# codeonwort/Software-Raytracing

Hardware: AMD Instinct MI355X
Metric: Mrays/sec (primary+secondary) + frame time, Cornell Box 1080p 64spp (higher is better)
Workload: dtype f32

## Files before the change

### include/raylib_amd.h

```cpp
#ifndef RAYLIB_AMD_H
#define RAYLIB_AMD_H

#include "raylib_types.h"

#ifdef __cplusplus
extern "C" {
#endif

typedef struct RaylibAMDStats {
	uint64_t rays;
	uint64_t nodesVisited;
	uint64_t trisTested;
	uint64_t shadedHits;
	uint64_t texFetches;
	uint64_t cameraSamples;
	uint64_t pixels;
	double   kernelMs;
	double   traceKernelMs;
	double   wallMs;
	uint32_t traceLaunches;
	uint32_t numNodes;
	uint32_t numTriangles;
	uint32_t bvhDepth;
	uint64_t waveTrips;
// ... 156 lines not shown

RAYLIB_API int32_t RaylibAMD_VerifyExactMath(int32_t which, uint64_t* outMismatches, uint64_t* outFirstBits);
RAYLIB_API int32_t RaylibAMD_VerifyLazyRefl(uint32_t n, uint64_t seed, uint64_t* outEvents, uint64_t* outUnsafe, uint64_t* outGuardFailed);
RAYLIB_API int32_t RaylibAMD_VerifyLazyPdf(uint32_t n, uint64_t seed, uint64_t* outEvents, uint64_t* outWrong, uint64_t* outRefused);

RAYLIB_API int32_t RaylibAMD_SceneNumTriangles(SceneHandle scene);
RAYLIB_API int32_t RaylibAMD_SceneNumMaterials(SceneHandle scene);
RAYLIB_API int32_t RaylibAMD_SceneNumTextures(SceneHandle scene);
RAYLIB_API void    RaylibAMD_SceneExportTriangles(SceneHandle scene, void* outTriangles);
RAYLIB_API void    RaylibAMD_SceneExportMaterials(SceneHandle scene, void* outMaterials);
RAYLIB_API void    RaylibAMD_SceneTextureSize(SceneHandle scene, int32_t index, int32_t* outW, int32_t* outH);
RAYLIB_API void    RaylibAMD_SceneExportTexture(SceneHandle scene, int32_t index, float* outRGBA);
RAYLIB_API void    RaylibAMD_SceneGetSun(SceneHandle scene, float outIlluminance[3], float outDirection[3]);
RAYLIB_API int32_t RaylibAMD_SceneBVHInfo(SceneHandle scene, uint32_t* outNodes, uint32_t* outDepth, float* outSahCost);
RAYLIB_API int32_t RaylibAMD_SceneBVH4Info(SceneHandle scene, uint32_t* outNodes4, uint32_t* outWorstCaseStack);
RAYLIB_API int32_t RaylibAMD_SceneBVH8Info(SceneHandle scene, uint32_t* outNodes8, uint32_t* outLevels, float* outSteps4, float* outSteps8);
RAYLIB_API int32_t RaylibAMD_SceneWalk8Host(SceneHandle scene, const float* rays, int32_t count, float tMin, const float* tMax, float* outT, uint32_t* outSteps);
RAYLIB_API int32_t RaylibAMD_SceneWalkStackHost(SceneHandle scene, int32_t tree, const float* rays, int32_t count, float tMin, int32_t capacity, float* outT, uint32_t* outHighWater);
RAYLIB_API int32_t RaylibAMD_SceneLeafListInfo(SceneHandle scene, uint32_t* outMaxTrianglesPerLeaf);
RAYLIB_API int32_t RaylibAMD_ScenePlain(SceneHandle scene);
RAYLIB_API int32_t RaylibAMD_LastTracePlain(void);
RAYLIB_API int32_t RaylibAMD_SceneLazyRefl(SceneHandle scene);
RAYLIB_API int32_t RaylibAMD_LastTraceLazy(void);
typedef struct RaylibAMDRenderPlan {
	int32_t pathTrace;
	int32_t stack, prims;
	int32_t poolK;
	int32_t tree;
	int32_t lstack;
	int32_t lds;
	int32_t plain;
	uint32_t pathsPerWave, treeWidth, nodeBytes;
	int32_t keepNodes4, keepNodes4f;
	int32_t eagerTree;
	uint32_t batch, sampleCount, blocks, stackStride, jobChunk, heads, jobsPerHead, guideShift;
	uint64_t jobs;
	int32_t lazy;
	int32_t reserved;
} RaylibAMDRenderPlan;
RAYLIB_API int32_t RaylibAMD_PlanRender(SceneHandle scene, const RendererSettings* settings, int32_t hasSky, int32_t numCUs, int32_t workgroupsPerCU, RaylibAMDRenderPlan* out);
#define RAYLIB_AMD_MAX_VIEWS 64
RAYLIB_API int32_t RaylibAMD_RenderViews(const RendererSettings* settings, SceneHandle scene,
        const CameraHandle* cameras, int32_t count, const ImageHandle* outImages);
RAYLIB_API int32_t RaylibAMD_RenderViewsDevice(const RendererSettings* settings, SceneHandle scene,
        const CameraHandle* cameras, int32_t count, void* outDevice);
RAYLIB_API int32_t RaylibAMD_PlanViews(SceneHandle scene, const RendererSettings* settings, const CameraHandle* cameras, int32_t count, int32_t hasSky,
// ... 43 lines not shown
```

### software-raytracing_amd/csrc/rl_abi.cc

```cpp
#include "raylib.h"
#include "raylib_amd.h"
#include "rl_host.h"
#include "rl_plan.h"
#include "rl_progressive.h"
#include "rl_lightmap.h"
#include "raylib_amd_rng.h"

#include <math.h>
#include <stddef.h>
#include <stdio.h>
#include <stdlib.h>
#include <string.h>
#include <algorithm>

using namespace rl;

namespace {

template <typename T>
struct Registry {
	std::mutex mu;
	std::vector<T*> items;
	void add(T* p) { std::lock_guard<std::mutex> lk(mu); items.push_back(p); }
	bool eraseFirst(T* p) {
// ... 1040 lines not shown
	return WalkStackHost(s->bvh, s->triangles, s->spheres, s->cubes, tree, rays, count, tMin, capacity, outT, outHighWater) ? 1 : -1;
}
int32_t RaylibAMD_SceneLeafListInfo(SceneHandle sh, uint32_t* maxPerLeaf)
{
	Scene* s = (Scene*)sh;
	if (!s || !s->finalized) return 0;
	int32_t leaves = 0; uint32_t most = 0;
	for (const DNode4& n : s->bvh.leafList) for (int k = 0; k < 4; ++k) if (n.child[k] != DNODE_EMPTY) { ++leaves; most = std::max(most, (((uint32_t)~n.child[k]) & LEAF_COUNT_MASK) + 1u); }
	if (maxPerLeaf) *maxPerLeaf = most;
	return leaves;
}
int32_t RaylibAMD_ScenePlain(SceneHandle sh)
{
	Scene* s = (Scene*)sh;
	return (s && s->finalized && ScenePlain(*s)) ? 1 : 0;
}
int32_t RaylibAMD_LastTracePlain(void) { return DeviceLastTracePlain(); }
int32_t RaylibAMD_SceneLazyRefl(SceneHandle sh)
{
	Scene* s = (Scene*)sh;
	return (s && s->finalized && SceneLazyRefl(*s)) ? 1 : 0;
}
int32_t RaylibAMD_LastTraceLazy(void) { return DeviceLastTraceLazy(); }
int32_t RaylibAMD_PlanRender(SceneHandle sh, const RendererSettings* settings, int32_t hasSky, int32_t numCUs, int32_t workgroupsPerCU, RaylibAMDRenderPlan* out)
{
	Scene* s = (Scene*)sh;
	if (!s || !s->finalized || !settings || !out || numCUs < 1) return 0;
	memset(out, 0, sizeof(*out));
	const RenderKnobs knobs = ReadRenderKnobs();
	const TracePlan t = PlanTrace(*s, *settings, hasSky != 0, knobs);
	if (!t.ok) return -1;
	out->pathTrace = t.pathTrace; out->stack = t.stack; out->prims = t.prims; out->poolK = t.poolK; out->tree = t.tree; out->lstack = t.lstack; out->lds = t.lds; out->plain = t.plain; out->lazy = t.lazy ? 1 : 0;
	out->pathsPerWave = t.pathsPerWave; out->treeWidth = t.treeWidth; out->nodeBytes = t.nodeBytes;
	out->keepNodes4 = t.keepNodes4; out->keepNodes4f = t.keepNodes4f; out->eagerTree = t.eagerTree;
	const uint32_t cells = ((settings->viewportWidth + 7) / 8) * ((settings->viewportHeight + 7) / 8);
	const uint32_t spp = (uint32_t)(settings->samplesPerPixel > 1 ? settings->samplesPerPixel : 1);
	const LaunchPlan L = PlanLaunch(cells, cells, spp, 0, numCUs, workgroupsPerCU, t, knobs);
	out->batch = L.batch; out->sampleCount = L.sampleCount; out->blocks = L.blocks; out->stackStride = L.stackStride; out->jobChunk = L.jobChunk;
	out->heads = L.heads; out->jobsPerHead = L.jobsPerHead; out->guideShift = L.guideShift; out->jobs = L.jobs;
	return 1;
}
int32_t RaylibAMD_PlanViews(SceneHandle sh, const RendererSettings* settings, const CameraHandle* cameras, int32_t count, int32_t hasSky,
                           int32_t numCUs, int32_t workgroupsPerCU, RaylibAMDRenderPlan* out, uint8_t* outCellEmpty)
{
	Scene* s = (Scene*)sh;
	if (!out || numCUs < 1 || !ViewsArgsValid("RaylibAMD_PlanViews", settings, s, cameras, count, nullptr)) return 0;
// ... 81 lines not shown
```

### software-raytracing_amd/csrc/rl_device.h

```cpp
#pragma once

#include <stdint.h>

namespace rl {

#define DNODE_EMPTY ((int32_t)0x80000000)
enum : uint32_t { LEAF_FIRST_SHIFT = 6, LEAF_KIND_SHIFT = 4, LEAF_KIND_MASK = 3u, LEAF_ALPHA_BIT = 8u, LEAF_COUNT_MASK = 7u };
struct alignas(64) DNode {
	float lmin[3], lmax[3];
	float rmin[3], rmax[3];
	int32_t left, right;
	int32_t pad0, pad1;
};
static_assert(sizeof(DNode) == 64, "DNode");

struct alignas(128) DNode4 {
	float lo[3][4];
	float hi[3][4];
	int32_t child[4];
	uint32_t pad[4];
};
static_assert(sizeof(DNode4) == 128, "DNode4");

struct alignas(64) DNode4Q {
// ... 156 lines not shown
	float    emptyL[3];
	uint32_t emptySky;
	uint32_t magicSamples;
	uint32_t magicCellsX;
	uint64_t seedMixed;
	DCamera camera;
};

#define RL_MAX_VIEWS 64
struct DViews {
	const DCamera* cameras;
	uint32_t cellsPerView;
	uint32_t magicCellsPerView;
};

#define RL_LIT_CHUNK 64u
#define RL_LIT_CTL 16u
#define RL_LAZY_ROUGHNESS_MIN 0x1p-10f
#define RL_LAZY_ROUGHNESS_MAX 1.0f
#define RL_LAZY_COLOR_MAX 16.0f
#define RL_LAZY_MAX_PATH 4096
#define RL_LAZY_REC_EXACT_SP 0x40000000
#define RL_LAZY_REC_MAT(w) (__float_as_int(w) & ~RL_LAZY_REC_EXACT_SP)
struct DLitList {
	float* entries;
	uint32_t* ctl;
	uint32_t numChunks;
	uint32_t pad;
};

}
```

### software-raytracing_amd/csrc/rl_host.h

```cpp
#pragma once

#include "raylib_types.h"
#include "raylib_amd.h"
#include "rl_device.h"

#include <math.h>
#include <stdint.h>
#include <memory>
#include <mutex>
#include <string>
#include <vector>

namespace rl {

struct f3 { float x, y, z; };
inline f3 F3(float x, float y, float z) { f3 r; r.x = x; r.y = y; r.z = z; return r; }
inline f3 operator+(f3 a, f3 b) { return F3(a.x + b.x, a.y + b.y, a.z + b.z); }
inline f3 operator-(f3 a, f3 b) { return F3(a.x - b.x, a.y - b.y, a.z - b.z); }
inline f3 operator*(f3 a, f3 b) { return F3(a.x * b.x, a.y * b.y, a.z * b.z); }
inline f3 operator*(f3 a, float t) { return F3(a.x * t, a.y * t, a.z * t); }
inline f3 operator*(float t, f3 a) { return F3(a.x * t, a.y * t, a.z * t); }
inline f3 operator-(f3 a) { return F3(-a.x, -a.y, -a.z); }
inline float dot(f3 a, f3 b) { return a.x * b.x + a.y * b.y + a.z * b.z; }
inline f3 cross(f3 a, f3 b) { return F3(a.y * b.z - a.z * b.y, -(a.x * b.z - a.z * b.x), a.x * b.y - a.y * b.x); }
// ... 153 lines not shown
	DCamera camera;
	uint64_t seed;
	uint32_t cellFirst, cellStride;
	bool cellMajor = false;
	int slot = 0;
	void* outDevice;
	bool callerOwnsOut = false;
	float* outHostRGBA;
};
bool DeviceAvailable();
int DeviceNumRanks();
float ParseDecimalFloat(const char* token);
constexpr uint64_t kMaxImagePixels = 1ull << 28;
inline bool PlausibleImageSize(uint64_t w, uint64_t h, uint64_t fileBytes, uint64_t maxPixelsPerByte)
{
	return w > 0 && h > 0 && w <= 65535 && h <= 65535 && w * h <= kMaxImagePixels && w * h <= (fileBytes + 64) * maxPixelsPerByte;
}
bool DecodeJPEG(const std::vector<uint8_t>& data, uint32_t& w, uint32_t& h, std::vector<uint8_t>& rgba);
bool DecodeTGA(const std::vector<uint8_t>& data, uint32_t& w, uint32_t& h, std::vector<uint8_t>& rgba);
bool EncodeJPEG(uint32_t w, uint32_t h, const uint8_t* rgbTopDown, std::vector<uint8_t>& out);
bool DeviceRender(Scene& scene, const RenderRequest& req, RaylibAMDStats& stats);
bool DeviceRenderViews(Scene& scene, const RenderRequest& req, const DCamera* cameras, uint32_t count, void* outDevice, void* const* imagePixels, RaylibAMDStats& stats);
int32_t DeviceLastTraceLazy();
int32_t DeviceLastTracePlain();
bool DeviceDrain(RaylibAMDStats* outLastStats);
void DeviceOwnStats();
bool DeviceClosestHit(Scene& scene, const float* rays, int32_t n, float tMin, void* outHits);
bool DeviceTraceRays(Scene& scene, int32_t kind, const void* rays, int32_t n, float rayTime, void* out, int32_t* outPrim, bool hostMem, void* stream,
                     RaylibAMDStats& stats);
constexpr uint64_t RL_RADIANCE_STACK_BUDGET = 256ull << 20;
constexpr int32_t RL_RADIANCE_MAX_PATH = 32768;
bool DeviceTraceRadiance(Scene& scene, const RaylibAMDRadianceParams& prm, uint64_t seed, const void* rays, int32_t n, float* out, bool hostMem, void* stream,
                         RaylibAMDStats& stats);
constexpr uint64_t RL_GATHER_SAMPLE_BUDGET = 256ull << 20;
constexpr uint64_t RL_GATHER_MAX_SLOTS = 1ull << 28;
constexpr uint64_t RL_GATHER_TIMED = 4096;
bool DeviceGather(Scene& scene, int32_t kind, const RaylibAMDRadianceParams& prm, uint64_t seed, const void* points, int32_t n, float* out, bool hostMem, void* stream,
                  RaylibAMDStats& stats);
int64_t LightmapPointsHost(const Scene& scene, const RaylibAMDLightmapParams& P, int32_t triFirst, int32_t triCount, const float* uv,
                           RaylibAMDGatherPoint* outPoints, uint32_t* outTexel, int64_t capacity);
int64_t DeviceLightmapPoints(Scene& scene, const RaylibAMDLightmapParams& P, int32_t triFirst, int32_t triCount, const float* uv,
                             RaylibAMDGatherPoint* outPoints, uint32_t* outTexel, int64_t capacity);
bool DeviceBakeLightmap(Scene& scene, const RaylibAMDLightmapParams& P, int32_t triFirst, int32_t triCount, const RaylibAMDRadianceParams& prm, uint64_t seed,
                        const float* uv, float* out, uint8_t* outCoverage, bool hostMem, void* stream, RaylibAMDStats& stats,
                        const RaylibAMDLightmapFilterParams* filter = nullptr, const float* in = nullptr);
struct LmFilterInv { float invC[8], invN, invP[8]; };
// ... 33 lines not shown
```

### software-raytracing_amd/csrc/rl_kernels.h

```cpp
#pragma once

#include "rl_dev_jobs.h"
#include "rl_dev_pool.h"

namespace rl {

#ifndef RL_QUEUE_SPIN_LIMIT
#define RL_QUEUE_SPIN_LIMIT 0
#endif
#ifndef RL_TRACE_MIN_WAVES
#define RL_TRACE_MIN_WAVES 4
#endif
#define RL_TRACE_ARGS const DRenderParams, const DSceneView, const SkyRot, SampleRGB* __restrict__, float* __restrict__, unsigned long long* __restrict__, unsigned int* __restrict__
template <int STACK, bool PRIMS, bool FULL, int LDS = 0, bool PLAIN = false>
__global__ void __launch_bounds__(RL_BLOCK, (STACK <= 32 ? RL_TRACE_MIN_WAVES : 2)) k_trace(RL_TRACE_ARGS);
template <int STACK, bool PRIMS, bool FULL, int LDS = 0, bool PLAIN = false>
__global__ void __launch_bounds__(RL_BLOCK, (STACK <= 32 ? RL_TRACE_MIN_WAVES : 2)) k_trace_views(RL_TRACE_ARGS, const DViews);
#define RL_TRACE_INSTANCES(X) \
	X(16, false, false, 0, false) X(16, false, true, 0, false) X(16, false, true, 1, false) X(16, false, true, 2, false) X(16, false, true, 2, true) \
	X(32, false, false, 0, false) X(32, false, true, 0, false) X(32, true, false, 0, false) X(32, true, true, 0, false) \
	X(64, false, false, 0, false) X(64, false, true, 0, false) X(64, true, false, 0, false) X(64, true, true, 0, false)
#define RL_K_TRACE(a, b, c, d, e) template __global__ void k_trace<a, b, c, d, e>(RL_TRACE_ARGS);
#define RL_K_TRACE_VIEWS(a, b, c, d, e) template __global__ void k_trace_views<a, b, c, d, e>(RL_TRACE_ARGS, const DViews);
RL_TRACE_INSTANCES(extern RL_K_TRACE)
RL_TRACE_INSTANCES(extern RL_K_TRACE_VIEWS)
template <int STACK, bool PRIMS, bool FULL, int LDS, bool PLAIN>
__global__ void __launch_bounds__(RL_BLOCK, (STACK <= 32 ? RL_TRACE_MIN_WAVES : 2)) k_trace_lazy(RL_TRACE_ARGS, const DLitList);
#define RL_TRACE_LAZY_INSTANCES(X) X(16, false, true, 2, true)
#define RL_K_TRACE_LAZY(a, b, c, d, e) template __global__ void k_trace_lazy<a, b, c, d, e>(RL_TRACE_ARGS, const DLitList);
RL_TRACE_LAZY_INSTANCES(extern RL_K_TRACE_LAZY)
__global__ void __launch_bounds__(RL_BLOCK) k_fold_lit(const DSceneView S, const DLitList LL, SampleRGB* __restrict__ samples);

template <int STACK, bool PRIMS, int K, int LSTACK = STACK, int WIDE = 0>
__global__ void __launch_bounds__(RL_BLOCK, (PoolOcc<LSTACK, PRIMS, K>::kBlocks)) k_trace_pool(RL_TRACE_ARGS);
template <int STACK, bool PRIMS, int K, int LSTACK = STACK, int WIDE = 0>
__global__ void __launch_bounds__(RL_BLOCK, (PoolOcc<LSTACK, PRIMS, K>::kBlocks)) k_trace_pool_views(RL_TRACE_ARGS, const DViews);
#define RL_POOL_INSTANCES(X) \
	X(16, false, 2, 16, 0) X(16, false, 3, 16, 0) X(16, false, 4, 16, 0) X(32, false, 2, 32, 0) X(32, false, 3, 32, 0) X(32, false, 4, 32, 0) \
	X(32, false, 2, 4, 0) X(32, false, 2, RL_POOL_SHORT_LSTACK, 0) \
	X(32, false, 2, 32, 1) X(64, false, 2, 32, 1) X(32, false, 2, RL_POOL_SHORT_LSTACK, 1) X(64, false, 2, RL_POOL_SHORT_LSTACK, 1) \
	X(2 * RL_POOL8_MAXLEVELS, false, 2, RL_POOL8_LSTACK, 3)
#define RL_K_TRACE_POOL(a, b, c, d, e) template __global__ void k_trace_pool<a, b, c, d, e>(RL_TRACE_ARGS);
#define RL_K_TRACE_POOL_VIEWS(a, b, c, d, e) template __global__ void k_trace_pool_views<a, b, c, d, e>(RL_TRACE_ARGS, const DViews);
RL_POOL_INSTANCES(extern RL_K_TRACE_POOL_VIEWS)
RL_POOL_INSTANCES(extern RL_K_TRACE_POOL)

__global__ void __launch_bounds__(RL_BLOCK)
k_resolve(const DRenderParams P, const DSceneView S, const SkyRot R, const SampleRGB* __restrict__ samples, float4* __restrict__ accum, float4* __restrict__ out, int firstBatch, int lastBatch);
__global__ void __launch_bounds__(RL_BLOCK)
k_resolve_views(const DRenderParams Pb, const DSceneView S, const SkyRot R, const SampleRGB* __restrict__ samples, float4* __restrict__ accum, float4* __restrict__ out,
                int firstBatch, int lastBatch, const DViews V);
#define RL_AOV_ARGS const DRenderParams, const DSceneView, float4* __restrict__, unsigned long long* __restrict__
template <int STACK, bool PRIMS> __global__ void __launch_bounds__(RL_BLOCK) k_aov(RL_AOV_ARGS);
template <int STACK, bool PRIMS> __global__ void __launch_bounds__(RL_BLOCK) k_aov_views(RL_AOV_ARGS, const DViews);
// ... 125 lines not shown
```

### software-raytracing_amd/csrc/rl_plan.cc

```cpp
#include "rl_plan.h"

#include <algorithm>
#include <atomic>
#include <cmath>
#include <cstring>
#include <stdlib.h>

namespace rl {

RenderKnobs ReadRenderKnobs()
{
	RenderKnobs k;
	auto flag = [](const char* name) { const char* e = getenv(name); return e ? (atoi(e) != 0 ? 1 : 0) : -1; };
	if (const char* e = getenv("RAYLIB_POOL")) { const int v = atoi(e); k.pool = (v == 2 || v == 3 || v == 4) ? v : 0; }
	if (const char* e = getenv("RAYLIB_POOL_MIN_TRIS")) k.poolMinTris = (uint32_t)atoi(e);
	if (const char* e = getenv("RAYLIB_POOL_SHORT_STACK")) { const int v = atoi(e); k.poolShortStack = (v == 0 || v == 4) ? v : 1; }
	k.bvh4 = flag("RAYLIB_BVH4"); k.bvh8 = flag("RAYLIB_BVH8");
	k.ldsScene = flag("RAYLIB_LDS_SCENE"); k.leafList = flag("RAYLIB_LEAF_LIST"); k.plainKernel = flag("RAYLIB_PLAIN_KERNEL");
	if (const char* e = getenv("RAYLIB_SAMPLE_BATCH")) k.sampleBatch = std::max(0, atoi(e));
	if (const char* e = getenv("RAYLIB_SAMPLE_BUFFER_GIB")) k.sampleBufferGiB = std::max(0, atoi(e));
	if (const char* e = getenv("RAYLIB_JOB_CHUNK")) k.jobChunk = std::max(0, atoi(e));
	if (const char* e = getenv("RAYLIB_JOB_HEADS")) k.jobHeads = std::max(1, atoi(e));
	if (const char* e = getenv("RAYLIB_GUIDED")) k.guided = atoi(e);
	if (const char* e = getenv("RAYLIB_BLOCKS_PER_CU")) k.blocksPerCU = std::max(0, atoi(e));
	if (const char* e = getenv("RAYLIB_CULL_CELLS")) k.cullCells = atoi(e);
	k.lazyRefl = flag("RAYLIB_LAZY_REFL");
	if (const char* e = getenv("RAYLIB_LIT_LIST")) k.litList = std::max(0ll, atoll(e));
	if (const char* e = getenv("RAYLIB_QUERY_TREE")) { const int v = atoi(e); k.queryTree = (v == 2 || v == 4 || v == 8) ? v : 0; }
	if (const char* e = getenv("RAYLIB_GATHER_BATCH")) k.gatherBatch = std::max(0, atoi(e));
	return k;
}

namespace {

TracePlan Pick(const Scene& sc, const RendererSettings& st, bool hasSky, const RenderKnobs& k, bool say)
{
	TracePlan p;
	const BVH& b = sc.bvh;
	const size_t ntri = sc.triangles.size();
	p.prims = !sc.spheres.empty() || !sc.cubes.empty();
	if (b.depth > 64) {
		if (say) Log("Raylib_Render: BVH depth %u exceeds the traversal stack (64)", b.depth);
		p.ok = false;
		return p;
	}
	p.stack = (b.depth <= 16 && !p.prims) ? 16 : b.depth <= 32 ? 32 : 64;
	p.pathTrace = st.renderMode == RAYLIB_RENDERMODE_Default;
	if (!p.pathTrace) return p;
	const bool hasNodes4 = !b.nodes4.empty(), hasNodes8 = !b.nodes8.empty();

// ... 224 lines not shown
```

### software-raytracing_amd/csrc/rl_plan.h

```cpp
#pragma once

#include "rl_host.h"

namespace rl {

#define RL_POOL_DEFAULT_MIN_TRIS 256u
#define RL_FLOAT_BOX_MAX_TRIS 4096u

struct RenderKnobs {
	int pool = -1;
	uint32_t poolMinTris = RL_POOL_DEFAULT_MIN_TRIS;
	int poolShortStack = -1;
	int bvh4 = -1, bvh8 = -1;
	int ldsScene = -1, leafList = -1, plainKernel = -1;
	int sampleBatch = 0, sampleBufferGiB = 0;
	int jobChunk = -1;
	int jobHeads = 0;
	int guided = 0;
	int blocksPerCU = 0;
	int cullCells = 1;
	int queryTree = 0;
	int gatherBatch = 0;
	int lazyRefl = -1;
	long long litList = -1;
};
RenderKnobs ReadRenderKnobs();

enum PlanTree : int32_t { TREE_NONE = 0, TREE_BVH2 = 1, TREE_BOX4 = 2, TREE_GRID4 = 3, TREE_WIDE8 = 4 };

struct TracePlan {
	bool ok = true;
	bool pathTrace = true;
	int stack = 16;
	bool prims = false;
	int poolK = 0;
	int32_t tree = TREE_BVH2;
	int lstack = 0;
	int lds = 0;
	bool plain = false;
	bool lazy = false;
	uint32_t pathsPerWave = 64, treeWidth = 2, nodeBytes = 64;
	bool keepNodes4 = true, keepNodes4f = true;
	int32_t eagerTree = TREE_NONE;
};
TracePlan PlanTrace(const Scene& sc, const RendererSettings& st, bool hasSky, const RenderKnobs& knobs);
int32_t EagerTree(const Scene& sc);

// ... 43 lines not shown
```

### software-raytracing_amd/csrc/rl_render_lazy.hip

```cpp


#include "rl_kernels.h"

namespace rl {

#define RL_VIEWS_TWIN 0
#define RL_LAZY_REFL 1
#include "rl_k_trace.inl"
#undef RL_LAZY_REFL
#undef RL_VIEWS_TWIN

__global__ void __launch_bounds__(RL_BLOCK)
k_fold_lit(const DSceneView S, const DLitList LL, SampleRGB* __restrict__ samples)
{
	RL_MATH_PROLOGUE();
	const uint32_t lane = threadIdx.x & 63u;
	const uint32_t waves = gridDim.x * (RL_BLOCK / 64u);
	const uint32_t used = min(LL.ctl[0], LL.numChunks);
	for (uint32_t chunk = (blockIdx.x * RL_BLOCK + threadIdx.x) >> 6; chunk < used; chunk += waves) {
		if (lane >= min(LL.ctl[RL_LIT_CTL + chunk], RL_LIT_CHUNK)) continue;
		const float4* e = (const float4*)LL.entries + ((size_t)chunk * RL_LIT_CHUNK + lane) * RL_LIT_STRIDE;
		const float4 h0 = e[0];
		const int nrec = __float_as_int(e[1].x);
		V3 L = v3(h0.x, h0.y, h0.z);
		#pragma nounroll
		for (int k = nrec - 1; k >= 0; --k) {
			const float4 r0 = e[2 + 2 * k], r1 = e[3 + 2 * k];
			L = FoldLazyVertex(LoadMat(S, RL_LAZY_REC_MAT(r1.w)), r0, r1, L);
		}
		samples[__float_as_uint(h0.w)] = make_sample(L.x, L.y, L.z);
	}
}

__device__ __forceinline__ uint32_t LazySweepEvent(unsigned long long seed, uint32_t i, Rng& g, V3& Wo, float& u0, float& u1, float& rough)
{
	g.s = raylib_rng_begin(seed, i, 0);
	const uint32_t sel = i % 30030u;
	const uint32_t zk = sel % 11u;
	float z = 2.0f * Next(g) - 1.0f;
	if (zk < 8u) { const float e[8] = { 0.0f, 1.0f, -1.0f, 0x1p-1f, -0x1p-10f, 0x1p-24f, -0x1p-60f, 0x1p-126f }; z = e[zk]; }
	const float phi = 2.0f * RL_PI * Next(g), rxy = rtm::sqrt_(fmaxf(0.0f, 1.0f - z * z));
	float sphi, cphi; rtm::sincos_(phi, &sphi, &cphi);
	Wo = v3(rxy * cphi, rxy * sphi, z);
	const uint32_t uk = sel % 7u, vk = sel % 5u;
	u0 = Next(g); u1 = Next(g);
	if (uk < 3u) u0 = uk == 0u ? 0.0f : uk == 1u ? 1e-6f : 1.0f - 0x1p-24f;
	if (vk < 3u) u1 = vk == 0u ? 0.0f : vk == 1u ? 1e-6f : 1.0f - 0x1p-24f;
	const uint32_t rk = sel % 3u;
	rough = rk == 0u ? RL_LAZY_ROUGHNESS_MIN : rk == 1u ? RL_LAZY_ROUGHNESS_MAX : rtm::exp_(Next(g) * -10.0f * 0.69314718f);
	return sel;
}

__global__ void __launch_bounds__(RL_BLOCK)
// ... 82 lines not shown
```

### software-raytracing_amd/csrc/rl_rt.h

```cpp
#pragma once

#include "rl_kernels.h"
#include "rl_plan.h"

#include <algorithm>
#include <chrono>
#include <condition_variable>
#include <functional>
#include <map>
#include <mutex>
#include <thread>

namespace rl {

#define HIP_OK(expr) do { hipError_t e_ = (expr); if (e_ != hipSuccess) { \
	Log("HIP error %s at %s:%d: %s", hipGetErrorName(e_), __FILE__, __LINE__, #expr); return false; } } while (0)
#define HIP_TRY(expr) do { hipError_t e_ = (expr); if (e_ != hipSuccess) { \
	Log("HIP error %s at %s:%d: %s", hipGetErrorName(e_), __FILE__, __LINE__, #expr); ok = false; } } while (0)

template <typename T, bool PINNED = false>
struct DevBuf {
	T* ptr = nullptr;
	size_t bytes = 0;
	DevBuf() = default;
// ... 86 lines not shown
				const bool r = f();
				{ std::lock_guard<std::mutex> lk(m); result = r; pending = false; }
				cv.notify_all();
			}
		}).detach();
	}
	void Post(std::function<bool()> f) { { std::lock_guard<std::mutex> lk(m); job = std::move(f); pending = true; } cv.notify_all(); }
	bool Wait() { std::unique_lock<std::mutex> lk(m); cv.wait(lk, [&] { return !pending; }); return result; }
};

#define RL_QUERY_RING 64
struct RankCtx {
	int rank = 0, device = 0, devSlot = 0, numCUs = 0;
	hipStream_t stream = nullptr;
	hipEvent_t ev[2][8] = {};
	PinBuf<unsigned long long> cntHost[2];
	DevBuf<SampleRGB> samples;
	DevBuf<float4> accum, image;
	DevBuf<float> pathStack;
	DevBuf<float4> cells;
	DevBuf<unsigned long long> counters;
	DevBuf<unsigned int> jobCounter;
	DevBuf<float4> litList; DevBuf<uint32_t> litCtl;
	PinBuf<uint32_t> cellListHost[2]; DevBuf<uint32_t> cellList[2]; size_t cellListCells[2] = { 0, 0 };
	std::vector<unsigned char> cullKey[2];
	uint32_t cullActive[2] = { 0, 0 }; uint64_t cullEmptyPixels[2] = { 0, 0 }; float cullL[2][3] = { { 0, 0, 0 }, { 0, 0, 0 } }; uint32_t cullRays[2] = { 1, 1 };
	std::map<const void*, int> occupancy;
	Worker* worker = nullptr;
	DevBuf<float4> qRays;
	DevBuf<void> qOut;
	DevBuf<int32_t> qPrim;
	DevBuf<unsigned int> qRing; hipEvent_t qRingEv[RL_QUERY_RING] = {}; bool qRingUsed[RL_QUERY_RING] = {}; uint32_t qRingNext = 0;
	DevBuf<unsigned long long> qStats; PinBuf<unsigned long long> qStatsHost;
	hipEvent_t qEv[2] = { nullptr, nullptr };
	DevBuf<unsigned int> radCounter;
	DevBuf<float> radStack;
	hipEvent_t radEv = nullptr; bool radEvUsed = false;
	DevBuf<float4> gSamples;
	DevBuf<float> gAcc;
	std::vector<hipEvent_t> gEv;
	DevBuf<DLmTri> lmRec; DevBuf<unsigned long long> lmCounts, lmSums; DevBuf<float> lmUv;
	DevBuf<uint32_t> lmOwner, lmRank, lmTexel; DevBuf<float4> lmPoints; DevBuf<float> lmValues, lmFilt, lmAtlas[2]; DevBuf<uint8_t> lmCov[2];
	PinBuf<unsigned long long> lmHost;
	hipEvent_t lmEv[6] = {};
	hipEvent_t lmInEv = nullptr;
};
// ... 57 lines not shown
```

### software-raytracing_amd/csrc/rl_rt_frame.hip

```cpp
#include "rl_rt.h"

#include <atomic>

namespace rl {

typedef void (*TraceKernel)(const DRenderParams, const DSceneView, const SkyRot, SampleRGB*, float*, unsigned long long*, unsigned int*);
typedef void (*TraceViewsKernel)(const DRenderParams, const DSceneView, const SkyRot, SampleRGB*, float*, unsigned long long*, unsigned int*, const DViews);
typedef void (*TraceLazyKernel)(const DRenderParams, const DSceneView, const SkyRot, SampleRGB*, float*, unsigned long long*, unsigned int*, const DLitList);
typedef void (*AovKernel)(const DRenderParams, const DSceneView, float4*, unsigned long long*);
typedef void (*AovViewsKernel)(const DRenderParams, const DSceneView, float4*, unsigned long long*, const DViews);

template <int STACK, bool PRIMS, bool FULL, int LDS = 0, bool PLAIN = false>
static const void* Trace(bool views)
{
	return views ? (const void*)(TraceViewsKernel)k_trace_views<STACK, PRIMS, FULL, LDS, PLAIN> : (const void*)(TraceKernel)k_trace<STACK, PRIMS, FULL, LDS, PLAIN>;
}
template <int STACK, bool PRIMS>
static const void* TraceFor(bool floatBoxes, bool views) { return floatBoxes ? Trace<STACK, PRIMS, true>(views) : Trace<STACK, PRIMS, false>(views); }
template <int STACK, bool PRIMS>
static const void* Aov(bool views) { return views ? (const void*)(AovViewsKernel)k_aov_views<STACK, PRIMS> : (const void*)(AovKernel)k_aov<STACK, PRIMS>; }
static const void* KernelFor(const TracePlan& p, bool views)
{
	if (p.poolK > 0) {
		const int wide = p.tree == TREE_WIDE8 ? 3 : p.tree == TREE_GRID4 ? 1 : 0;
// ... 1 lines not shown
			return views ? (const void*)(TraceViewsKernel)k_trace_pool_views<a, b, c, d, e> : (const void*)(TraceKernel)k_trace_pool<a, b, c, d, e>;
		RL_POOL_INSTANCES(RL_POOL_PICK)
#undef RL_POOL_PICK
		return nullptr;
	}
	if (p.lds == 2 && p.lazy && !views) return (const void*)(TraceLazyKernel)k_trace_lazy<16, false, true, 2, true>;
	if (p.lds == 2) return p.plain ? Trace<16, false, true, 2, true>(views) : Trace<16, false, true, 2>(views);
	if (p.lds == 1) return Trace<16, false, true, 1>(views);
	const bool full = p.tree == TREE_BOX4;
	if (p.stack == 16) return TraceFor<16, false>(full, views);
	if (p.stack == 32) return p.prims ? TraceFor<32, true>(full, views) : TraceFor<32, false>(full, views);
	return p.prims ? TraceFor<64, true>(full, views) : TraceFor<64, false>(full, views);
}
static const void* AovKernelFor(const TracePlan& p, bool views)
{
	if (p.stack == 16) return Aov<16, false>(views);
	if (p.stack == 32) return p.prims ? Aov<32, true>(views) : Aov<32, false>(views);
	return p.prims ? Aov<64, true>(views) : Aov<64, false>(views);
}
static std::atomic<int32_t> g_lastTracePlain{0};
int32_t DeviceLastTracePlain() { return g_lastTracePlain.load(std::memory_order_relaxed); }
static std::atomic<int32_t> g_lastTraceLazy{0};
int32_t DeviceLastTraceLazy() { return g_lastTraceLazy.load(std::memory_order_relaxed); }

struct Frame {
	RenderKnobs knobs;
	TracePlan plan;
	DSceneView view;
	DRenderParams P;
	uint32_t numLive = 0, numActive = 0;
	uint32_t sBegin = 0, sEnd = 1;
	float4* out = nullptr;
	const DViews* views = nullptr;
	const void* resolve = nullptr;
	void* resolveArgs[5] = {};
	int firstBatch = 0, lastBatch = 0;
	bool accum = true;
	ProgressiveSession* compact = nullptr;
};

static DRenderParams BaseParams(const RendererSettings& st, uint64_t seed, const DCamera& camera, uint32_t cellFirst, uint32_t stride, uint32_t numLocalCells, bool rowMajor)
{
	DRenderParams P; memset(&P, 0, sizeof(P));
	const uint32_t W = st.viewportWidth, H = st.viewportHeight, cellsX = (W + 7) / 8;
	P.width = W; P.height = H; P.spp = (uint32_t)(st.samplesPerPixel > 1 ? st.samplesPerPixel : 1); P.maxPathLength = st.maxPathLength; P.rayTMin = st.rayTMin;
	P.invWidth = 1.0f / (float)W; P.invHeight = 1.0f / (float)H;
// ... 50 lines not shown
	DRenderParams& P = F.P;
	const uint32_t numCells = P.numLocalCells, numSlots = numCells * 64u;
	const uint32_t rblocks = (numSlots + RL_BLOCK - 1) / RL_BLOCK;
	SkyRot skyRot = DS.skyRot;
	if (numSlots == 0) {
	} else if (!plan.pathTrace) {
		void* args[] = { &P, &F.view, &F.out, &R.counters.ptr, (void*)F.views };
		HIP_OK(hipLaunchKernel(AovKernelFor(plan, F.views != nullptr), dim3(rblocks), dim3(RL_BLOCK), args, 0, R.stream));
	} else {
		const void* traceKernel = KernelFor(plan, F.views != nullptr);
		if (!traceKernel) { Log("Raylib_Render: no megakernel instance for STACK %d, K %d, stack in LDS %d", plan.stack, plan.poolK, plan.lstack); return false; }
		const int blocksPerCU = OccupancyOf(R, traceKernel, &plan);
		if (blocksPerCU < 0) return false;
		g_lastTracePlain.store(plan.plain ? 1 : 0, std::memory_order_relaxed);
		const bool lazy = plan.lazy && !F.views;
		g_lastTraceLazy.store(lazy ? 1 : 0, std::memory_order_relaxed);
		pend.lazy = lazy;
		DLitList LL = {};
		pend.pathsPerWave = plan.pathsPerWave; pend.treeWidth = plan.treeWidth; pend.nodeBytes = plan.nodeBytes;
		pend.culledCells = F.numLive - F.numActive; pend.listedCells = F.numActive;
		const uint32_t batch = PlanLaunch(numCells, F.numActive, F.sEnd, F.sBegin, R.numCUs, blocksPerCU, plan, F.knobs).batch;
		if (!R.samples.Grow((size_t)numSlots * sizeof(SampleRGB) * std::min(batch, F.sEnd - F.sBegin))) return false;
		if (F.accum && batch < P.spp && !R.accum.Grow((size_t)numSlots * sizeof(float4))) return false;
		const int depthSlots = P.maxPathLength > 1 ? P.maxPathLength : 1;
		void* traceArgs[] = { &P, &F.view, &skyRot, &R.samples.ptr, &R.pathStack.ptr, &R.counters.ptr, &R.jobCounter.ptr, lazy ? (void*)&LL : (void*)F.views };
		void* foldArgs[] = { &F.view, &LL, &R.samples.ptr };
		void* resolveArgs[] = { &P, &F.view, &skyRot, &R.samples.ptr, F.resolveArgs[0], F.resolveArgs[1], F.resolveArgs[2], F.resolveArgs[3], F.resolveArgs[4] };
		for (uint32_t s0 = F.sBegin; s0 < F.sEnd; s0 += batch) {
			const LaunchPlan L = PlanLaunch(numCells, F.numActive, F.sEnd, s0, R.numCUs, blocksPerCU, plan, F.knobs);
			const uint32_t cnt = L.sampleCount;
			P.sampleBegin = s0; P.sampleCount = cnt;
			P.magicSamples = cnt > 1 ? (uint32_t)(0x100000000ull / cnt) : 0xFFFFFFFFu;
			if (L.jobs > 0xF0000000ull) { Log("Raylib_Render: job count overflow"); return false; }
			P.numJobs = (uint32_t)L.jobs;
			P.stackStride = L.stackStride; P.jobChunk = L.jobChunk;
			P.numHeads = L.heads; P.jobsPerHead = L.jobsPerHead; P.guideShift = L.guideShift;
			if (!R.pathStack.Grow((size_t)depthSlots * 8 * P.stackStride * sizeof(float))) return false;
			if (lazy) {
				const uint64_t want = F.knobs.litList >= 0 ? (uint64_t)F.knobs.litList
				                                           : std::max<uint64_t>(4096, L.jobs / 32) + (uint64_t)L.blocks * (RL_BLOCK / 64) * RL_LIT_CHUNK;
				const uint32_t chunks = (uint32_t)std::min<uint64_t>(want / RL_LIT_CHUNK, 0x7FFFFFFFu / RL_LIT_CHUNK);
				if (!R.litList.Grow(std::max<size_t>(1, chunks) * RL_LIT_CHUNK * RL_LIT_STRIDE * sizeof(float4))) return false;
				if (!R.litCtl.Grow((RL_LIT_CTL + (size_t)chunks) * sizeof(uint32_t))) return false;
				LL.entries = (float*)R.litList.ptr; LL.ctl = R.litCtl.ptr; LL.numChunks = chunks;
				HIP_OK(hipMemsetAsync(R.litCtl.ptr, 0, (RL_LIT_CTL + (size_t)chunks) * sizeof(uint32_t), R.stream));
			}
			pend.jobHeads = L.heads;
			F.firstBatch = s0 == F.sBegin; F.lastBatch = s0 + cnt >= F.sEnd;
			HIP_OK(hipMemsetAsync(R.jobCounter.ptr, 0, RL_MAX_HEADS * RL_HEAD_STRIDE * sizeof(unsigned int), R.stream));
			HIP_OK(hipEventRecord(R.ev[q][2], R.stream));
			if (L.jobs > 0)
				HIP_OK(hipLaunchKernel(traceKernel, dim3(L.blocks), dim3(RL_BLOCK), traceArgs, 0, R.stream));
			if (L.jobs > 0 && lazy && LL.numChunks > 0)
				HIP_OK(hipLaunchKernel((const void*)k_fold_lit, dim3(std::min<uint32_t>((LL.numChunks + 3u) / 4u, (uint32_t)R.numCUs * 8u)), dim3(RL_BLOCK), foldArgs, 0, R.stream));
			HIP_OK(hipEventRecord(R.ev[q][3], R.stream));
			HIP_OK(hipLaunchKernel(F.resolve, dim3(rblocks), dim3(RL_BLOCK), resolveArgs, 0, R.stream));
			++pend.launches;
			if (!F.lastBatch) {
				HIP_OK(hipEventSynchronize(R.ev[q][3]));
				float ms = 0.0f;
				HIP_OK(hipEventElapsedTime(&ms, R.ev[q][2], R.ev[q][3]));
				pend.traceMs += ms;
			} else pend.lastBatchPending = true;
		}
		if (ProgressiveSession* S = F.compact) {
			hipLaunchKernelGGL(k_progressive_compact, dim3(1), dim3(RL_COMPACT_BLOCK), 0, R.stream,
			                   S->live.ptr, S->trace.ptr, (const uint8_t*)S->st.stopped, (const uint8_t*)S->empty.ptr, S->numLive, P.width, P.height, P.cellsX, S->counts.ptr);
			HIP_OK(hipGetLastError());
			HIP_OK(hipMemcpyAsync(S->countsHost.ptr, S->counts.ptr, 4 * sizeof(uint32_t), hipMemcpyDeviceToHost, R.stream));
		}
	}
	if (!plan.pathTrace) pend.listedCells = numCells;
	HIP_OK(hipEventRecord(R.ev[q][1], R.stream));
	HIP_OK(hipMemcpyAsync(R.cntHost[q].ptr, R.counters.ptr, (CNT_COUNT + 24) * sizeof(unsigned long long), hipMemcpyDeviceToHost, R.stream));
	if (pend.lazy) HIP_OK(hipMemcpyAsync(R.cntHost[q].ptr + CNT_COUNT + 24, R.counters.ptr + RL_CNT_LIT, 2 * sizeof(unsigned long long), hipMemcpyDeviceToHost, R.stream));
	HIP_OK(hipEventRecord(R.ev[q][7], R.stream));
	pend.enqueuedToEnd = true;
	return true;
}
// ... 242 lines not shown
```

### software-raytracing_amd/raylib_amd/binding.py

```python
import ctypes as C
import os
import numpy as np

HERE = os.path.dirname(os.path.abspath(__file__))
LIB_PATH = os.environ.get("RAYLIB_LIB") or os.path.join(os.path.dirname(HERE), "libraylib.so")

RENDERMODE_DEFAULT, RENDERMODE_ALBEDO, RENDERMODE_SURFACE_NORMAL, RENDERMODE_MICROSURFACE_NORMAL, \
    RENDERMODE_TEXCOORD, RENDERMODE_EMISSION, RENDERMODE_REFLECTANCE = range(7)


class RendererSettings(C.Structure):
    _fields_ = [("viewportWidth", C.c_uint32), ("viewportHeight", C.c_uint32),
                ("samplesPerPixel", C.c_int32), ("maxPathLength", C.c_int32),
                ("rayTMin", C.c_float), ("renderMode", C.c_uint32)]


class DenoiseParams(C.Structure):
    _fields_ = [("iterations", C.c_int32), ("sigmaColor", C.c_float), ("sigmaNormal", C.c_float), ("sigmaAlbedo", C.c_float)]


class ProgressiveParams(C.Structure):
    _fields_ = [("threshold", C.c_float), ("minSamples", C.c_uint32)]


# ... 437 lines not shown
                                                   C.POINTER(C.c_uint8), C.c_void_p]),
    "RaylibAMD_FilterLightmapHost": (C.c_int32, [C.c_int32, C.c_int32, C.c_int32, C.POINTER(LightmapFilterParams), C.POINTER(GatherPoint), C.POINTER(C.c_uint32), C.c_int64,
                                                 C.POINTER(C.c_float), C.POINTER(C.c_float)]),
    "RaylibAMD_VerifyExactMath": (C.c_int32, [C.c_int32, C.POINTER(C.c_uint64), C.POINTER(C.c_uint64)]),
    "RaylibAMD_CullCells": (C.c_int32, [C.c_void_p, C.POINTER(C.c_float), C.POINTER(C.c_float), C.POINTER(C.c_float), C.c_int32, C.c_int32, C.POINTER(C.c_uint8), C.POINTER(C.c_float)]),
    "RaylibAMD_SceneNumTriangles": (C.c_int32, [C.c_void_p]),
    "RaylibAMD_SceneNumMaterials": (C.c_int32, [C.c_void_p]),
    "RaylibAMD_SceneNumTextures": (C.c_int32, [C.c_void_p]),
    "RaylibAMD_SceneExportTriangles": (None, [C.c_void_p, C.c_void_p]),
    "RaylibAMD_SceneExportMaterials": (None, [C.c_void_p, C.c_void_p]),
    "RaylibAMD_SceneTextureSize": (None, [C.c_void_p, C.c_int32, C.POINTER(C.c_int32), C.POINTER(C.c_int32)]),
    "RaylibAMD_SceneExportTexture": (None, [C.c_void_p, C.c_int32, C.POINTER(C.c_float)]),
    "RaylibAMD_SceneGetSun": (None, [C.c_void_p, C.POINTER(C.c_float), C.POINTER(C.c_float)]),
    "RaylibAMD_SceneBVHInfo": (C.c_int32, [C.c_void_p, C.POINTER(C.c_uint32), C.POINTER(C.c_uint32), C.POINTER(C.c_float)]),
    "RaylibAMD_ParseFloat": (C.c_float, [C.c_char_p]),
    "RaylibAMD_ImageSize": (C.c_int32, [C.c_void_p, C.POINTER(C.c_uint32), C.POINTER(C.c_uint32)]),
    "RaylibAMD_SceneBVH4Info": (C.c_int32, [C.c_void_p, C.POINTER(C.c_uint32), C.POINTER(C.c_uint32)]),
    "RaylibAMD_SceneBVH8Info": (C.c_int32, [C.c_void_p, C.POINTER(C.c_uint32), C.POINTER(C.c_uint32), C.POINTER(C.c_float), C.POINTER(C.c_float)]),
    "RaylibAMD_SceneLeafListInfo": (C.c_int32, [C.c_void_p, C.POINTER(C.c_uint32)]),
    "RaylibAMD_ScenePlain": (C.c_int32, [C.c_void_p]),
    "RaylibAMD_LastTracePlain": (C.c_int32, []),
    "RaylibAMD_SceneLazyRefl": (C.c_int32, [C.c_void_p]),
    "RaylibAMD_LastTraceLazy": (C.c_int32, []),
    "RaylibAMD_VerifyLazyRefl": (C.c_int32, [C.c_uint32, C.c_uint64, C.POINTER(C.c_uint64), C.POINTER(C.c_uint64), C.POINTER(C.c_uint64)]),
    "RaylibAMD_VerifyLazyPdf": (C.c_int32, [C.c_uint32, C.c_uint64, C.POINTER(C.c_uint64), C.POINTER(C.c_uint64), C.POINTER(C.c_uint64)]),
    "RaylibAMD_PlanRender": (C.c_int32, [C.c_void_p, C.POINTER(RendererSettings), C.c_int32, C.c_int32, C.c_int32, C.POINTER(RenderPlan)]),
    "RaylibAMD_SceneWalk8Host": (C.c_int32, [C.c_void_p, C.POINTER(C.c_float), C.c_int32, C.c_float, C.POINTER(C.c_float), C.POINTER(C.c_float), C.POINTER(C.c_uint32)]),
    "RaylibAMD_SceneWalkStackHost": (C.c_int32, [C.c_void_p, C.c_int32, C.POINTER(C.c_float), C.c_int32, C.c_float, C.c_int32, C.POINTER(C.c_float), C.POINTER(C.c_uint32)]),
    "RaylibAMD_SceneBVHHash": (C.c_uint64, [C.c_void_p]),
    "RaylibAMD_CameraExport": (None, [C.c_void_p, C.POINTER(C.c_float)]),
    "RaylibAMD_CreateImageFromData": (C.c_void_p, [C.c_uint32, C.c_uint32, C.POINTER(C.c_float)]),
    "RaylibAMD_DumpImageRGBA": (None, [C.c_void_p, C.POINTER(C.c_float)]),
    "RaylibAMD_OBJModelSetTexture": (C.c_int32, [C.c_void_p, C.c_char_p, C.c_int32, C.c_void_p]),
    "RaylibAMD_Denoise": (C.c_int32, [C.c_void_p, C.c_int32, C.c_void_p, C.c_void_p, C.c_void_p, C.POINTER(DenoiseParams)]),
    "RaylibAMD_DenoiseHost": (C.c_int32, [C.c_uint32, C.c_uint32, C.POINTER(C.c_float), C.c_int32, C.POINTER(C.c_float), C.POINTER(C.c_float),
                                          C.POINTER(DenoiseParams), C.POINTER(C.c_float)]),
    "RaylibAMD_EnableDenoiser": (None, [C.c_int32]),
    "RaylibAMD_BeginProgressive": (C.c_size_t, [C.POINTER(RendererSettings), C.c_void_p, C.c_void_p, C.c_void_p, C.POINTER(ProgressiveParams)]),
    "RaylibAMD_ProgressiveStep": (C.c_int32, [C.c_size_t, C.c_uint32]),
    "RaylibAMD_ProgressiveExport": (C.c_int32, [C.c_size_t, C.POINTER(C.c_uint32), C.POINTER(C.c_uint8), C.POINTER(C.c_float), C.POINTER(C.c_float)]),
    "RaylibAMD_EndProgressive": (C.c_int32, [C.c_size_t]),
    "RaylibAMD_ProgressiveDecideHost": (C.c_int32, [C.c_uint32, C.c_uint32, C.POINTER(C.c_uint32), C.POINTER(C.c_float), C.POINTER(C.c_float),
                                                    C.POINTER(ProgressiveParams), C.POINTER(C.c_uint8)]),
    "RaylibAMD_ProgressiveCompactTest": (C.c_int32, [C.POINTER(C.c_uint32), C.c_uint32, C.POINTER(C.c_uint8), C.POINTER(C.c_uint8), C.c_uint32, C.c_uint32, C.c_uint32,
                                                     C.POINTER(C.c_uint32), C.POINTER(C.c_uint32), C.POINTER(C.c_uint32)]),
    "RaylibAMD_RenderViews": (C.c_int32, [C.POINTER(RendererSettings), C.c_void_p, C.POINTER(C.c_void_p), C.c_int32, C.POINTER(C.c_void_p)]),
# ... 254 lines not shown
```

Baseline: 19410.

## Add lit-sample bitmask so resolve sums only nonzero lazy samples

```diff
diff --git a/include/raylib_amd.h b/include/raylib_amd.h
--- a/include/raylib_amd.h
+++ b/include/raylib_amd.h
@@ -202,6 +202,7 @@
 RAYLIB_API int32_t RaylibAMD_LastTracePlain(void);
 RAYLIB_API int32_t RaylibAMD_SceneLazyRefl(SceneHandle scene);
 RAYLIB_API int32_t RaylibAMD_LastTraceLazy(void);
+RAYLIB_API int32_t RaylibAMD_LastLitMask(void);
 typedef struct RaylibAMDRenderPlan {
 	int32_t pathTrace;
 	int32_t stack, prims;
diff --git a/software-raytracing_amd/csrc/rl_abi.cc b/software-raytracing_amd/csrc/rl_abi.cc
--- a/software-raytracing_amd/csrc/rl_abi.cc
+++ b/software-raytracing_amd/csrc/rl_abi.cc
@@ -1086,6 +1086,7 @@
 	return (s && s->finalized && SceneLazyRefl(*s)) ? 1 : 0;
 }
 int32_t RaylibAMD_LastTraceLazy(void) { return DeviceLastTraceLazy(); }
+int32_t RaylibAMD_LastLitMask(void) { return DeviceLastLitMask(); }
 int32_t RaylibAMD_PlanRender(SceneHandle sh, const RendererSettings* settings, int32_t hasSky, int32_t numCUs, int32_t workgroupsPerCU, RaylibAMDRenderPlan* out)
 {
 	Scene* s = (Scene*)sh;
diff --git a/software-raytracing_amd/csrc/rl_device.h b/software-raytracing_amd/csrc/rl_device.h
--- a/software-raytracing_amd/csrc/rl_device.h
+++ b/software-raytracing_amd/csrc/rl_device.h
@@ -202,11 +202,13 @@
 #define RL_LAZY_MAX_PATH 4096
 #define RL_LAZY_REC_EXACT_SP 0x40000000
 #define RL_LAZY_REC_MAT(w) (__float_as_int(w) & ~RL_LAZY_REC_EXACT_SP)
+#define RL_LIT_MASK_MAX_WORDS 8u
 struct DLitList {
 	float* entries;
 	uint32_t* ctl;
 	uint32_t numChunks;
-	uint32_t pad;
+	uint32_t maskWords;
+	uint32_t* mask;
 };
 
 }
diff --git a/software-raytracing_amd/csrc/rl_host.h b/software-raytracing_amd/csrc/rl_host.h
--- a/software-raytracing_amd/csrc/rl_host.h
+++ b/software-raytracing_amd/csrc/rl_host.h
@@ -199,6 +199,7 @@
 bool DeviceRender(Scene& scene, const RenderRequest& req, RaylibAMDStats& stats);
 bool DeviceRenderViews(Scene& scene, const RenderRequest& req, const DCamera* cameras, uint32_t count, void* outDevice, void* const* imagePixels, RaylibAMDStats& stats);
 int32_t DeviceLastTraceLazy();
+int32_t DeviceLastLitMask();
 int32_t DeviceLastTracePlain();
 bool DeviceDrain(RaylibAMDStats* outLastStats);
 void DeviceOwnStats();
diff --git a/software-raytracing_amd/csrc/rl_kernels.h b/software-raytracing_amd/csrc/rl_kernels.h
--- a/software-raytracing_amd/csrc/rl_kernels.h
+++ b/software-raytracing_amd/csrc/rl_kernels.h
@@ -29,7 +29,10 @@
 #define RL_TRACE_LAZY_INSTANCES(X) X(16, false, true, 2, true)
 #define RL_K_TRACE_LAZY(a, b, c, d, e) template __global__ void k_trace_lazy<a, b, c, d, e>(RL_TRACE_ARGS, const DLitList);
 RL_TRACE_LAZY_INSTANCES(extern RL_K_TRACE_LAZY)
-__global__ void __launch_bounds__(RL_BLOCK) k_fold_lit(const DSceneView S, const DLitList LL, SampleRGB* __restrict__ samples);
+__global__ void __launch_bounds__(RL_BLOCK) k_fold_lit(const DSceneView S, const DLitList LL, SampleRGB* __restrict__ samples, uint32_t numSlots);
+__global__ void __launch_bounds__(RL_BLOCK)
+k_resolve_lit(const DRenderParams P, const DSceneView S, const SkyRot R, const SampleRGB* __restrict__ samples, float4* __restrict__ accum, float4* __restrict__ out,
+              int firstBatch, int lastBatch, const DLitList LL);
 
 template <int STACK, bool PRIMS, int K, int LSTACK = STACK, int WIDE = 0>
 __global__ void __launch_bounds__(RL_BLOCK, (PoolOcc<LSTACK, PRIMS, K>::kBlocks)) k_trace_pool(RL_TRACE_ARGS);
diff --git a/software-raytracing_amd/csrc/rl_lit_mask.h b/software-raytracing_amd/csrc/rl_lit_mask.h
--- /dev/null
+++ b/software-raytracing_amd/csrc/rl_lit_mask.h
@@ -0,0 +1,30 @@
+#pragma once
+
+#include <stddef.h>
+#include <stdint.h>
+
+#if defined(__HIPCC__)
+#define RL_LM_HD __host__ __device__ inline
+#else
+#define RL_LM_HD inline
+#endif
+
+namespace rl {
+
+RL_LM_HD size_t LitMaskWord(uint32_t s, uint32_t numSlots, uint32_t slot) { return (size_t)(s >> 5) * numSlots + slot; }
+RL_LM_HD uint32_t LitMaskBit(uint32_t s) { return 1u << (s & 31u); }
+
+RL_LM_HD void LitMaskSum(const uint32_t* mask, uint32_t maskWords, const float* samples, uint32_t numSlots, uint32_t slot, float& ax, float& ay, float& az)
+{
+	for (uint32_t w = 0; w < maskWords; ++w) {
+		uint32_t m = mask[(size_t)w * numSlots + slot];
+		while (m != 0u) {
+			const uint32_t s = w * 32u + (uint32_t)__builtin_ctz(m);
+			const float* v = samples + ((size_t)s * numSlots + slot) * 3u;
+			ax += v[0]; ay += v[1]; az += v[2];
+			m &= m - 1u;
+		}
+	}
+}
+
+}
diff --git a/software-raytracing_amd/csrc/rl_plan.cc b/software-raytracing_amd/csrc/rl_plan.cc
--- a/software-raytracing_amd/csrc/rl_plan.cc
+++ b/software-raytracing_amd/csrc/rl_plan.cc
@@ -26,6 +26,7 @@
 	if (const char* e = getenv("RAYLIB_CULL_CELLS")) k.cullCells = atoi(e);
 	k.lazyRefl = flag("RAYLIB_LAZY_REFL");
 	if (const char* e = getenv("RAYLIB_LIT_LIST")) k.litList = std::max(0ll, atoll(e));
+	k.litMask = flag("RAYLIB_LIT_MASK");
 	if (const char* e = getenv("RAYLIB_QUERY_TREE")) { const int v = atoi(e); k.queryTree = (v == 2 || v == 4 || v == 8) ? v : 0; }
 	if (const char* e = getenv("RAYLIB_GATHER_BATCH")) k.gatherBatch = std::max(0, atoi(e));
 	return k;
diff --git a/software-raytracing_amd/csrc/rl_plan.h b/software-raytracing_amd/csrc/rl_plan.h
--- a/software-raytracing_amd/csrc/rl_plan.h
+++ b/software-raytracing_amd/csrc/rl_plan.h
@@ -23,6 +23,7 @@
 	int gatherBatch = 0;
 	int lazyRefl = -1;
 	long long litList = -1;
+	int litMask = -1;
 };
 RenderKnobs ReadRenderKnobs();
 
diff --git a/software-raytracing_amd/csrc/rl_render_lazy.hip b/software-raytracing_amd/csrc/rl_render_lazy.hip
--- a/software-raytracing_amd/csrc/rl_render_lazy.hip
+++ b/software-raytracing_amd/csrc/rl_render_lazy.hip
@@ -1,6 +1,7 @@
 
 
 #include "rl_kernels.h"
+#include "rl_lit_mask.h"
 
 namespace rl {
 
@@ -11,7 +12,7 @@
 #undef RL_VIEWS_TWIN
 
 __global__ void __launch_bounds__(RL_BLOCK)
-k_fold_lit(const DSceneView S, const DLitList LL, SampleRGB* __restrict__ samples)
+k_fold_lit(const DSceneView S, const DLitList LL, SampleRGB* __restrict__ samples, uint32_t numSlots)
 {
 	RL_MATH_PROLOGUE();
 	const uint32_t lane = threadIdx.x & 63u;
@@ -28,7 +29,43 @@
 			const float4 r0 = e[2 + 2 * k], r1 = e[3 + 2 * k];
 			L = FoldLazyVertex(LoadMat(S, RL_LAZY_REC_MAT(r1.w)), r0, r1, L);
 		}
-		samples[__float_as_uint(h0.w)] = make_sample(L.x, L.y, L.z);
+		const uint32_t outIndex = __float_as_uint(h0.w);
+		if (!LL.mask) samples[outIndex] = make_sample(L.x, L.y, L.z);
+		else if (AnyBitSet(L)) {
+			const uint32_t s = outIndex / numSlots;
+			samples[outIndex] = make_sample(L.x, L.y, L.z);
+			atomicOr(&LL.mask[LitMaskWord(s, numSlots, outIndex - s * numSlots)], LitMaskBit(s));
+		}
+	}
+}
+
+__global__ void __launch_bounds__(RL_BLOCK)
+k_resolve_lit(const DRenderParams P, const DSceneView S, const SkyRot R, const SampleRGB* __restrict__ samples, float4* __restrict__ accum, float4* __restrict__ out,
+              int firstBatch, int lastBatch, const DLitList LL)
+{
+	RL_MATH_PROLOGUE();
+	const uint32_t numSlots = P.numLocalCells * 64u;
+	const uint32_t slot = blockIdx.x * RL_BLOCK + threadIdx.x;
+	if (slot >= numSlots) return;
+	const uint32_t p = slot & 63u, cellLocal = slot >> 6;
+	const uint32_t cell = P.cellFirst + cellLocal * P.cellStride;
+	const uint32_t x = (cell % P.cellsX) * 8u + (p & 7u), y = (cell / P.cellsX) * 8u + (p >> 3);
+	const bool valid = x < P.width && y < P.height;
+	float4 a = make_float4(0.0f, 0.0f, 0.0f, 1.0f);
+	if (valid) {
+		if (!firstBatch) a = accum[slot];
+		if (P.cellEmpty && P.cellEmpty[cellLocal]) a = SumSlotBatch(P, S, R, samples, numSlots, slot, cellLocal, x, y, a, [](float, float, float) __attribute__((always_inline)) {});
+		else LitMaskSum(LL.mask, LL.maskWords, (const float*)samples, numSlots, slot, a.x, a.y, a.z);
+		if (lastBatch) {
+			const float k = rtm::rcp1_((float)P.spp);
+			a.x *= k; a.y *= k; a.z *= k; a.w = 1.0f;
+		} else {
+			accum[slot] = a;
+		}
+	}
+	if (lastBatch) {
+		if (P.rowMajorOutput) { if (valid) out[(size_t)y * P.width + x] = a; }
+		else out[slot] = valid ? a : make_float4(0.0f, 0.0f, 0.0f, 0.0f);
 	}
 }
 
diff --git a/software-raytracing_amd/csrc/rl_rt.h b/software-raytracing_amd/csrc/rl_rt.h
--- a/software-raytracing_amd/csrc/rl_rt.h
+++ b/software-raytracing_amd/csrc/rl_rt.h
@@ -132,6 +132,7 @@
 	DevBuf<unsigned long long> counters;
 	DevBuf<unsigned int> jobCounter;
 	DevBuf<float4> litList; DevBuf<uint32_t> litCtl;
+	DevBuf<uint32_t> litMask;
 	PinBuf<uint32_t> cellListHost[2]; DevBuf<uint32_t> cellList[2]; size_t cellListCells[2] = { 0, 0 };
 	std::vector<unsigned char> cullKey[2];
 	uint32_t cullActive[2] = { 0, 0 }; uint64_t cullEmptyPixels[2] = { 0, 0 }; float cullL[2][3] = { { 0, 0, 0 }, { 0, 0, 0 } }; uint32_t cullRays[2] = { 1, 1 };
diff --git a/software-raytracing_amd/csrc/rl_rt_frame.hip b/software-raytracing_amd/csrc/rl_rt_frame.hip
--- a/software-raytracing_amd/csrc/rl_rt_frame.hip
+++ b/software-raytracing_amd/csrc/rl_rt_frame.hip
@@ -47,6 +47,8 @@
 int32_t DeviceLastTracePlain() { return g_lastTracePlain.load(std::memory_order_relaxed); }
 static std::atomic<int32_t> g_lastTraceLazy{0};
 int32_t DeviceLastTraceLazy() { return g_lastTraceLazy.load(std::memory_order_relaxed); }
+static std::atomic<int32_t> g_lastLitMask{0};
+int32_t DeviceLastLitMask() { return g_lastLitMask.load(std::memory_order_relaxed); }
 
 struct Frame {
 	RenderKnobs knobs;
@@ -143,10 +145,14 @@
 		const uint32_t batch = PlanLaunch(numCells, F.numActive, F.sEnd, F.sBegin, R.numCUs, blocksPerCU, plan, F.knobs).batch;
 		if (!R.samples.Grow((size_t)numSlots * sizeof(SampleRGB) * std::min(batch, F.sEnd - F.sBegin))) return false;
 		if (F.accum && batch < P.spp && !R.accum.Grow((size_t)numSlots * sizeof(float4))) return false;
+		const bool masked = lazy && F.resolve == (const void*)k_resolve && F.knobs.litMask != 0 && (F.knobs.litMask > 0 || !F.view.hasSun) &&
+		                    (std::min(batch, F.sEnd - F.sBegin) + 31u) / 32u <= RL_LIT_MASK_MAX_WORDS;
+		g_lastLitMask.store(masked ? 1 : 0, std::memory_order_relaxed);
+		const void* resolveKernel = masked ? (const void*)k_resolve_lit : F.resolve;
 		const int depthSlots = P.maxPathLength > 1 ? P.maxPathLength : 1;
 		void* traceArgs[] = { &P, &F.view, &skyRot, &R.samples.ptr, &R.pathStack.ptr, &R.counters.ptr, &R.jobCounter.ptr, lazy ? (void*)&LL : (void*)F.views };
-		void* foldArgs[] = { &F.view, &LL, &R.samples.ptr };
-		void* resolveArgs[] = { &P, &F.view, &skyRot, &R.samples.ptr, F.resolveArgs[0], F.resolveArgs[1], F.resolveArgs[2], F.resolveArgs[3], F.resolveArgs[4] };
+		void* foldArgs[] = { &F.view, &LL, &R.samples.ptr, (void*)&numSlots };
+		void* resolveArgs[] = { &P, &F.view, &skyRot, &R.samples.ptr, F.resolveArgs[0], F.resolveArgs[1], F.resolveArgs[2], F.resolveArgs[3], masked ? (void*)&LL : F.resolveArgs[4] };
 		for (uint32_t s0 = F.sBegin; s0 < F.sEnd; s0 += batch) {
 			const LaunchPlan L = PlanLaunch(numCells, F.numActive, F.sEnd, s0, R.numCUs, blocksPerCU, plan, F.knobs);
 			const uint32_t cnt = L.sampleCount;
@@ -165,6 +171,13 @@
 				if (!R.litCtl.Grow((RL_LIT_CTL + (size_t)chunks) * sizeof(uint32_t))) return false;
 				LL.entries = (float*)R.litList.ptr; LL.ctl = R.litCtl.ptr; LL.numChunks = chunks;
 				HIP_OK(hipMemsetAsync(R.litCtl.ptr, 0, (RL_LIT_CTL + (size_t)chunks) * sizeof(uint32_t), R.stream));
+				if (masked) {
+					const uint32_t words = (cnt + 31u) / 32u;
+					const size_t bytes = (size_t)words * numSlots * sizeof(uint32_t);
+					if (!R.litMask.Grow(bytes)) return false;
+					LL.mask = R.litMask.ptr; LL.maskWords = words;
+					HIP_OK(hipMemsetAsync(R.litMask.ptr, 0, bytes, R.stream));
+				}
 			}
 			pend.jobHeads = L.heads;
 			F.firstBatch = s0 == F.sBegin; F.lastBatch = s0 + cnt >= F.sEnd;
@@ -175,7 +188,7 @@
 			if (L.jobs > 0 && lazy && LL.numChunks > 0)
 				HIP_OK(hipLaunchKernel((const void*)k_fold_lit, dim3(std::min<uint32_t>((LL.numChunks + 3u) / 4u, (uint32_t)R.numCUs * 8u)), dim3(RL_BLOCK), foldArgs, 0, R.stream));
 			HIP_OK(hipEventRecord(R.ev[q][3], R.stream));
-			HIP_OK(hipLaunchKernel(F.resolve, dim3(rblocks), dim3(RL_BLOCK), resolveArgs, 0, R.stream));
+			HIP_OK(hipLaunchKernel(resolveKernel, dim3(rblocks), dim3(RL_BLOCK), resolveArgs, 0, R.stream));
 			++pend.launches;
 			if (!F.lastBatch) {
 				HIP_OK(hipEventSynchronize(R.ev[q][3]));
diff --git a/software-raytracing_amd/raylib_amd/binding.py b/software-raytracing_amd/raylib_amd/binding.py
--- a/software-raytracing_amd/raylib_amd/binding.py
+++ b/software-raytracing_amd/raylib_amd/binding.py
@@ -483,6 +483,7 @@
     "RaylibAMD_LastTracePlain": (C.c_int32, []),
     "RaylibAMD_SceneLazyRefl": (C.c_int32, [C.c_void_p]),
     "RaylibAMD_LastTraceLazy": (C.c_int32, []),
+    "RaylibAMD_LastLitMask": (C.c_int32, []),
     "RaylibAMD_VerifyLazyRefl": (C.c_int32, [C.c_uint32, C.c_uint64, C.POINTER(C.c_uint64), C.POINTER(C.c_uint64), C.POINTER(C.c_uint64)]),
     "RaylibAMD_VerifyLazyPdf": (C.c_int32, [C.c_uint32, C.c_uint64, C.POINTER(C.c_uint64), C.POINTER(C.c_uint64), C.POINTER(C.c_uint64)]),
     "RaylibAMD_PlanRender": (C.c_int32, [C.c_void_p, C.POINTER(RendererSettings), C.c_int32, C.c_int32, C.c_int32, C.POINTER(RenderPlan)]),
```

After: 19730, median of 6. 1.7% higher.
